# pureexe/deeparc-sfm

Hardware: AMD Instinct MI355X
Metric: M observations/sec residual+Jacobian; wall-clock/LM-iter at 1/2/4/8 GPUs (higher is better)
Workload: dtype f64; 1 GPU; c3_1kcam per GPU: 1000 cameras, 100000 points, 1000000 observations, BAL-shaped, eval pass = residual+Jacobian reduced into the JtJ/Jtr blocks; global_obs=1000000, parallelism=point-sharded x1, RCCL all-reduce of camera blocks

## Files before the change

### deeparc-sfm_amd/__init__.py

```python
from ._abi import (DAB_CONVERGENCE, DAB_E_INVALID, DAB_E_UNSUPPORTED, DAB_FAILURE, DAB_LINEAR_SOLVER_AUTO,
                   DAB_LINEAR_SOLVER_EXPLICIT_SCHUR, DAB_LINEAR_SOLVER_IMPLICIT_SCHUR_PCG, DAB_LOSS_CAUCHY,
                   DAB_LOSS_HUBER, DAB_LOSS_SOFT_L1, DAB_LOSS_TRIVIAL, DAB_NO_CONVERGENCE, LIB_PATH,
                   SIGNATURES, load_library, last_error)
from ._abi import DabCovarianceInfo, DabCovarianceIntrInfo, DabCovarianceOptions
from ._abi import DAB_INTR_CENTER, DAB_INTR_DISTORTION, DAB_INTR_FOCAL
from ._abi import DAB_EXT_ROTATION, DAB_EXT_TRANSLATION
from ._abi import DAB_SCHUR_DIRECT, DAB_SCHUR_PAIRS, DAB_SCHUR_TILES
from .core import (CONFIGS, Problem, Solver, covariance_options, options, point_sqrt_info_from_sigmas, solve,
                   sqrt_info_from_sigmas, synth, synth_config)

__all__ = [
    "CONFIGS", "Problem", "Solver", "options", "solve", "synth", "synth_config",
    "covariance_options", "DabCovarianceOptions", "DabCovarianceInfo", "DabCovarianceIntrInfo",
    "load_library", "last_error", "LIB_PATH", "SIGNATURES",
    "DAB_CONVERGENCE", "DAB_NO_CONVERGENCE", "DAB_FAILURE",
    "DAB_LINEAR_SOLVER_EXPLICIT_SCHUR", "DAB_LINEAR_SOLVER_IMPLICIT_SCHUR_PCG", "DAB_LINEAR_SOLVER_AUTO",
    "DAB_LOSS_TRIVIAL", "DAB_LOSS_HUBER", "DAB_LOSS_SOFT_L1", "DAB_LOSS_CAUCHY",
    "DAB_E_INVALID", "DAB_E_UNSUPPORTED",
    "DAB_INTR_CENTER", "DAB_INTR_FOCAL", "DAB_INTR_DISTORTION",
    "DAB_EXT_ROTATION", "DAB_EXT_TRANSLATION",
    "DAB_SCHUR_PAIRS", "DAB_SCHUR_TILES", "DAB_SCHUR_DIRECT",
    "sqrt_info_from_sigmas", "point_sqrt_info_from_sigmas",
]
```

### deeparc-sfm_amd/_abi.py

```python
import ctypes as C
import os

HERE = os.path.dirname(os.path.abspath(__file__))
LIB_PATH = os.path.join(HERE, "libdab.so")

DAB_OK = 0
DAB_LINEAR_SOLVER_EXPLICIT_SCHUR = 0
DAB_LINEAR_SOLVER_IMPLICIT_SCHUR_PCG = 1
DAB_LINEAR_SOLVER_AUTO = 2
DAB_CONVERGENCE = 0
DAB_NO_CONVERGENCE = 1
DAB_FAILURE = 2
TERMINATION = {0: "CONVERGENCE", 1: "NO_CONVERGENCE", 2: "FAILURE"}
DAB_E_INVALID = -1
DAB_E_UNSUPPORTED = -6
DAB_LOSS_TRIVIAL = 0
DAB_LOSS_HUBER = 1
DAB_LOSS_SOFT_L1 = 2
DAB_LOSS_CAUCHY = 3
DAB_INTR_CENTER = 1
DAB_INTR_FOCAL = 2
DAB_INTR_DISTORTION = 4
DAB_EXT_ROTATION = 0x07
DAB_EXT_TRANSLATION = 0x38
# ... 143 lines not shown
    "dab_eval_intr_priors": (C.c_int, [C.c_void_p, _dp, _dp]),
    "dab_get_intrinsics": (C.c_int, [C.c_void_p, _dp]),
    "dab_update_intrinsics": (C.c_int, [C.c_void_p, _dp]),
    "dab_eval_intrinsic_jacobians": (C.c_int, [C.c_void_p, _dp]),
    "dab_get_intrinsic_blocks": (C.c_int, [C.c_void_p, _ip, _dp]),
    "dab_covariance_options_init": (None, [C.POINTER(DabCovarianceOptions)]),
    "dab_covariance": (C.c_int, [C.c_void_p, C.POINTER(DabCovarianceOptions), _dp, _dp, _dp,
                                 C.POINTER(DabCovarianceInfo)]),
    "dab_covariance_intrinsics": (C.c_int, [C.c_void_p, C.POINTER(DabCovarianceOptions), _dp, _dp, _dp, _dp,
                                            C.POINTER(DabCovarianceInfo), C.POINTER(DabCovarianceIntrInfo)]),
    "dab_eval_residuals": (C.c_int, [C.c_void_p, _dp, _dp]),
    "dab_eval_jacobians": (C.c_int, [C.c_void_p, _dp, _dp]),
    "dab_filter": (C.c_int, [C.c_void_p, C.c_double, _dp, C.c_double, _u8p, _u8p, _ip, _ip]),
    "dab_dense_spd_solve": (C.c_int, [C.c_void_p, C.c_int, _dp, _dp, _dp, _dp]),
    "dab_bench_eval_pass": (C.c_int, [C.c_void_p, C.c_int, C.c_int]),
    "dab_sync": (C.c_int, [C.c_void_p]),
    "dab_bench_get_blocks": (C.c_int, [C.c_void_p, _ip, _ip, _dp, _dp, _dp, _dp, _dp]),
    "dab_bench_kernel_ms": (C.c_int, [C.c_void_p, _dp, _dp]),
    "dab_jacobian_bytes": (C.c_int, [C.c_void_p, _dp]),
    "dab_bench_pair_ms": (C.c_int, [C.c_void_p, _dp, _dp]),
    "dab_eval_schedule": (C.c_int, [C.c_void_p, _ip]),
    "dab_pcg_schedule": (C.c_int, [C.c_void_p, _ip]),
    "dab_comm_schedule": (C.c_int, [C.c_void_p, _ip]),
    "dab_synth_sizes": (C.c_int, [C.POINTER(DabSynthConfig), _ip, _ip, _ip, _ip]),
    "dab_synth_fill": (C.c_int, [C.POINTER(DabSynthConfig), C.POINTER(DabProblem), _u8p]),
}

_LIB = None


def load_library(path=None):
    global _LIB
    if _LIB is not None and path is None:
        return _LIB
    p = path or LIB_PATH
    if not os.path.exists(p):
        raise RuntimeError(
            f"libdab.so not found at {p}: build it with `make -C deeparc-sfm_amd` "
            "(hipcc --offload-arch=gfx950). There is no CPU fallback.")
    lib = C.CDLL(p)
    for name, (res, args) in SIGNATURES.items():
        fn = getattr(lib, name)
        fn.restype = res
        fn.argtypes = args
    if lib.dab_abi_version() != 2:
        raise RuntimeError("libdab ABI version mismatch")
# ... 16 lines not shown
```

### deeparc-sfm_amd/core.py

```python
import ctypes as C

import numpy as np

from . import _abi
from ._abi import (DabOptions, DabProblem, DabSummary, DabIteration, DabSynthConfig,
                   DabCovarianceOptions, DabCovarianceInfo, DabCovarianceIntrInfo, check, load_library)


def _ptr(a, ct):
    return a.ctypes.data_as(C.POINTER(ct)) if a is not None else None


class Problem:

    def __init__(self, obs_xy, obs_point, obs_ext0, obs_ext1, obs_intr, points, ext, intr,
                 intr_nf, intr_nk, ext_const=None, freeze_camera=False):
        self.obs_xy = np.ascontiguousarray(obs_xy, dtype=np.float64).reshape(-1, 2)
        self.obs_point = np.ascontiguousarray(obs_point, dtype=np.int32)
        self.obs_ext0 = np.ascontiguousarray(obs_ext0, dtype=np.int32)
        self.obs_ext1 = np.ascontiguousarray(obs_ext1, dtype=np.int32)
        self.obs_intr = np.ascontiguousarray(obs_intr, dtype=np.int32)
        self.points = np.ascontiguousarray(points, dtype=np.float64).reshape(-1, 3)
        self.ext = np.ascontiguousarray(ext, dtype=np.float64).reshape(-1, 6)
        self.intr = np.ascontiguousarray(intr, dtype=np.float64).reshape(-1, 6)
# ... 545 lines not shown
        return b.value

    def bench_pair_ms(self):
        a, b = C.c_double(), C.c_double()
        check(self.lib.dab_bench_pair_ms(self.h, C.byref(a), C.byref(b)), self.lib)
        return a.value, b.value

    def comm_p2p(self):
        f = C.c_int32()
        check(self.lib.dab_comm_schedule(self.h, C.byref(f)), self.lib)
        return int(f.value)

    def pcg_matrix_free(self):
        f = C.c_int32()
        check(self.lib.dab_pcg_schedule(self.h, C.byref(f)), self.lib)
        return int(f.value)

    def eval_fused(self):
        f = C.c_int32()
        check(self.lib.dab_eval_schedule(self.h, C.byref(f)), self.lib)
        return f.value


def sqrt_info_from_sigmas(sigma_w, sigma_t, n=None):
    def inv(sg):
        return 0.0 if sg is None or np.isinf(sg) else 1.0 / float(sg)
    a = np.diag([inv(sigma_w)] * 3 + [inv(sigma_t)] * 3)
    return a if n is None else np.repeat(a[None], int(n), axis=0)


def point_sqrt_info_from_sigmas(sigma, n=None):
    sg = [sigma] * 3 if sigma is None or np.ndim(sigma) == 0 else list(sigma)
    if len(sg) != 3:
        raise ValueError("sigma: a scalar or 3 values")
    a = np.diag([0.0 if v is None or np.isinf(v) else 1.0 / float(v) for v in sg])
    return a if n is None else np.repeat(a[None], int(n), axis=0)


def solve(problem, max_iteration=1000, max_second=3600, freeze_camera=False, device=0,
          verbose=False, loss=None, free_intrinsics=0, freeze_points=False, ext_priors=None, point_priors=None,
          intr_priors=None, ext_scalars_constant=None, **opt_kw):
    problem.freeze_camera = bool(freeze_camera)
    o = options(max_num_iterations=max_iteration, max_solver_time_in_seconds=float(max_second),
                minimizer_progress_to_stdout=int(verbose), **opt_kw)
    s = Solver(device)
    try:
# ... 19 lines not shown
```

### deeparc-sfm_amd/csrc/dab_handle.h

```cpp
#pragma once
#include <hip/hip_runtime.h>
#include <rccl/rccl.h>

#include <algorithm>
#include <limits>
#include <array>
#include <chrono>
#include <climits>
#include <cmath>
#include <cstdio>
#include <cstdlib>
#include <cstring>
#include <string>
#include <thread>
#include <vector>

#include "dab_devmem.h"
#include "dab_internal.h"
#include "dab_kernels.h"
#include "dab_p2p.h"
#include "dab_setup.h"

#define HIP_OK(expr)                                                                           \
  do {                                                                                         \
// ... 127 lines not shown
  S_SYNC,
  S_SYNC1,
  S_ZPRIOR,
  S_NSLOTS
};


template <class T, class A>
int upload(T** dptr, Dev& dev, const std::vector<T, A>& h, hipStream_t s) {
  CHECK_RC(dev.alloc(dptr, h.size()));
  if (!h.empty()) HIP_OK(hipMemcpyAsync(*dptr, h.data(), h.size() * sizeof(T), hipMemcpyHostToDevice, s));
  return 0;
}

struct Knobs {
  int chunk = 0;
  int xchunk = 0;
  int pair_eval = -1;
  int eval_wps = INT_MIN;
  int eval_fused = 1;
  int eval_split = 0;
  int pcg_fused = 1;
  int pcg_mf = 1;
  int cg_onewg = 0;
  int bench_sample = 8;
  int schur_tiles = 1;
  int tile_balance = 1;
  int tile_single = 1;
  int tile_minb = 2;
  int p2p = -1;
  int intr_border_lds = 1;
  int setup_host = 0;
  int eval_side = 0;
  int fused_tab = -1;
  int points_direct = 1;
  void read() {
    auto get = [](const char* name, int& out) {
      if (const char* e = getenv(name)) out = atoi(e);
    };
    get("DAB_CHUNK", chunk);
    get("DAB_XCHUNK", xchunk);
    get("DAB_PAIR_EVAL", pair_eval);
    get("DAB_EVAL_WPS", eval_wps);
    get("DAB_EVAL_FUSED", eval_fused);
    get("DAB_EVAL_SPLIT", eval_split);
    get("DAB_PCG_FUSED", pcg_fused);
    get("DAB_PCG_MF", pcg_mf);
    get("DAB_CG_ONEWG", cg_onewg);
    get("DAB_BENCH_SAMPLE", bench_sample);
    get("DAB_SCHUR_TILES", schur_tiles);
    get("DAB_TILE_BALANCE", tile_balance);
    get("DAB_TILE_MINB", tile_minb);
    get("DAB_TILE_SINGLE", tile_single);
    get("DAB_P2P", p2p);
    get("DAB_FUSED_TAB", fused_tab);
    get("DAB_SETUP_HOST", setup_host);
    get("DAB_INTR_BORDER_LDS", intr_border_lds);
    get("DAB_EVAL_SIDE", eval_side);
    get("DAB_POINTS_DIRECT", points_direct);
  }
  bool eval_side_ok() const {
#ifdef DAB_ABLATIONS
    return eval_side >= 0 && eval_side <= 7;
#else
    return eval_side == 0 || eval_side == 7;
#endif
  }
};

struct PhaseTimer {
// ... 35 lines not shown
  bool any_compose = false;
  std::vector<int> perm;
  std::vector<int> pt_of;
  std::vector<int> ext_col;
  int nchunk = 0, nxchunk = 0, ncross = 0, nblk = 0, nslice = 0;
  int max_seg_chunks = 1, max_xseg_chunks = 1;
  int NS = 0;
  long long npairs = 0;
  int lds = 0;
  bool schur_built = false;
  bool pcg_built = false;
  int nxlist = 0;
  std::vector<int> h_pt_ent_ptr;
  big_vec<int> h_ent_cam, h_ent_pos, h_ent_os;

  Dev dev{"problem buffers"};
  Dev setup_tmp{"set-up scratch"};
  Dev keep_dev{"kept buffers"};
  DevView view{};
  double loss_scale = 0.0;
  int4* d_obs_idx = nullptr;
  double2* d_obs_xy = nullptr;
  int* d_obs_e = nullptr;
  int4* d_cm_idx = nullptr;
  double2* d_cm_xy = nullptr;
  int4* d_x_idx = nullptr;
  double2* d_x_xy = nullptr;
  int *d_slice_off = nullptr, *d_pt_ent_ptr = nullptr, *d_ent_os = nullptr, *d_ent_cam = nullptr,
      *d_ent_pt = nullptr, *d_ent_pos = nullptr, *d_cm_pt = nullptr, *d_ext_col = nullptr;
  int *d_chunk_beg = nullptr, *d_seg_chunk = nullptr;
  int2* d_chunk_uni = nullptr;
  int uni_affine = 0, uni_ox = 0, uni_oi = 0;
  unsigned* d_arrivals = nullptr;
  int* d_chunk_lists = nullptr;
  ChunkLists chunks;
  int *d_xchunk_beg = nullptr, *d_xseg_chunk = nullptr;
  int2* d_cross_cam = nullptr;
  int2 *d_pairs = nullptr, *d_blk_cam = nullptr;
  int2* d_blk_zero = nullptr;
  int nzero = 0;
  int* d_blk_pair_beg = nullptr;
  double* d_intr = nullptr;
  std::vector<uint8_t> intr_mask;
  std::vector<uint8_t> intr_ref;
  bool intr_ref_union = false;
  std::vector<double> intr_host;
// ... 340 lines not shown
```

### deeparc-sfm_amd/csrc/dab_handle.hip

```cpp
#include <map>
#include <mutex>

#include "dab_handle.h"
#include "dab_warm.h"

using namespace dab;

namespace dab {
namespace {
std::mutex& cache_mu() {
  static std::mutex* m = new std::mutex();
  return *m;
}
std::map<int, std::vector<hipStream_t>>& stream_cache() {
  static auto* c = new std::map<int, std::vector<hipStream_t>>();
  return *c;
}
std::map<size_t, std::vector<void*>>& pinned_cache() {
  static auto* c = new std::map<size_t, std::vector<void*>>();
  return *c;
}
}
hipStream_t stream_take(int device) {
  {
// ... 329 lines not shown
  if (!h || !h->have_problem) return set_error(DAB_E_STATE, "no problem set");
  HIP_OK(hipSetDevice(h->device));
  if (points) {
    std::vector<double> pts((size_t)3 * h->NP);
    HIP_OK(hipMemcpyAsync(pts.data(), h->d_points, pts.size() * sizeof(double), hipMemcpyDeviceToHost, h->stream));
    HIP_OK(hipStreamSynchronize(h->stream));
    for (int i = 0; i < h->NP; ++i)
      for (int k = 0; k < 3; ++k) points[3 * (size_t)h->pt_of[i] + k] = pts[3 * (size_t)i + k];
  }
  if (ext) {
    HIP_OK(hipMemcpyAsync(ext, h->d_ext, sizeof(double) * 6 * (size_t)h->E, hipMemcpyDeviceToHost, h->stream));
    HIP_OK(hipStreamSynchronize(h->stream));
  }
  return 0;
}

extern "C" int dab_comm_schedule(dab_handle* h, int32_t* p2p) {
  clear_error();
  if (!h || !p2p) return set_error(DAB_E_INVALID, "null argument");
  *p2p = (h->p2p_main || h->p2p_comm) ? 1 : 0;
  return 0;
}

extern "C" int dab_pcg_schedule(dab_handle* h, int32_t* matrix_free) {
  clear_error();
  if (!h || !h->have_problem || !matrix_free) return set_error(DAB_E_STATE, "no problem set");
  *matrix_free = h->pcg_built && h->mf ? (h->mf32 ? 2 : 1) : 0;
  return 0;
}

extern "C" int dab_eval_schedule(dab_handle* h, int32_t* fused) {
  clear_error();
  if (!h || !h->have_problem || !fused) return set_error(DAB_E_STATE, "no problem set");
  *fused = h->fused ? (h->fused_split ? 2 : 1) : 0;
  return 0;
}
```

### deeparc-sfm_amd/csrc/dab_k_step.hip

```cpp
#include <hip/hip_runtime.h>

#include <algorithm>

#include "dab_kernels.h"
#include "dab_reduce.h"
#include "dab_rows.h"
#include "dab_warm.h"
#include "dab_wave.h"

namespace dab {

__global__ __launch_bounds__(256) void k_point_factor(DevView v, const double* __restrict__ V,
                                                      const double* __restrict__ g,
                                                      const double* __restrict__ sp, StepScalars sc,
                                                      double* __restrict__ L, double* __restrict__ q,
                                                      int* __restrict__ fail) {
  const int p = blockIdx.x * blockDim.x + threadIdx.x;
  if (p >= v.NP) return;
  const size_t NPs = (size_t)v.NP;
  const double s0 = sp[p], s1 = sp[NPs + p], s2 = sp[2 * NPs + p];
  double v00 = s0 * V[p] * s0, v01 = s0 * V[NPs + p] * s1, v02 = s0 * V[2 * NPs + p] * s2;
  double v11 = s1 * V[3 * NPs + p] * s1, v12 = s1 * V[4 * NPs + p] * s2, v22 = s2 * V[5 * NPs + p] * s2;
  auto lmd = [&](double d) {
    d = fmin(fmax(d, sc.min_diag), sc.max_diag);
    const double D = sqrt(d / sc.radius);
    return D * D;
  };
  v00 += lmd(v00);
  v11 += lmd(v11);
  v22 += lmd(v22);
  bool ok = v00 > 0.0;
// ... 367 lines not shown
#pragma unroll
      for (int slot = 0; slot < 2; ++slot) {
        const int e = slot ? id.z : id.y;
        const int c = e >= 0 ? v.ext_col[e] : -1;
        if (c < 0) continue;
        double y[18];
        load_yplane(Ypm + slot * 18 * NS, NS, (size_t)s, y);
#pragma unroll
        for (int a = 0; a < 6; ++a) {
          const double ycv = yc[6 * c + a];
          r[0] -= y[3 * a] * ycv;
          r[1] -= y[3 * a + 1] * ycv;
          r[2] -= y[3 * a + 2] * ycv;
        }
      }
    }
  }
  const double* pu = PU + 6 * (size_t)p;
  dp[p] = -(pu[0] * r[0] + pu[1] * r[1] + pu[2] * r[2]);
  dp[NPs + p] = -(pu[3] * r[1] + pu[4] * r[2]);
  dp[2 * NPs + p] = -(pu[5] * r[2]);
}

void launch_backsub(hipStream_t s, const DevView& v, const double* PU, const double* q, YBufs Y,
                    const double* yc, double* delta_p) {
  if (v.NP <= 0) return;
  const int g = grid_for(v.NP, 256, 1 << 20);
  if (Y.f32) k_backsub<float><<<g, 256, 0, s>>>(v, PU, q, (const float*)Y.pm, yc, delta_p);
  else k_backsub<double><<<g, 256, 0, s>>>(v, PU, q, (const double*)Y.pm, yc, delta_p);
}

__global__ __launch_bounds__(256) void k_axpy_points(int NP, const double* __restrict__ x,
                                                     const double* __restrict__ d,
                                                     double* __restrict__ xc, double* __restrict__ partial) {
  double acc[2] = {0.0, 0.0};
  const size_t NPs = (size_t)NP;
  for (int i = blockIdx.x * blockDim.x + threadIdx.x; i < 3 * NP; i += gridDim.x * blockDim.x) {
    const int p = i / 3, k = i - 3 * (i / 3);
    const double xv = x[i];
    const double c = xv + d[k * NPs + p];
    xc[i] = c;
    const double dd = xv - c;
    acc[0] += dd * dd;
    acc[1] += c * c;
  }
  block_reduce_store<2>(acc, partial + 2 * (size_t)blockIdx.x);
}

void launch_axpy_points(hipStream_t s, int NP, const double* x, const double* d, double* xc,
                        double* partial, int grid) {
// ... 61 lines not shown
```

### deeparc-sfm_amd/csrc/dab_kernels.h

```cpp
#pragma once
#include <string>
#include <hip/hip_runtime.h>

#include <cstdint>

#include "../../include/dab.h"

namespace dab {

#define DAB_LOSS_SWITCH(loss_, ...)                                                          \
  switch (loss_) {                                                                           \
    case DAB_LOSS_HUBER: { constexpr int LOSS = DAB_LOSS_HUBER; __VA_ARGS__; } break;         \
    case DAB_LOSS_SOFT_L1: { constexpr int LOSS = DAB_LOSS_SOFT_L1; __VA_ARGS__; } break;     \
    case DAB_LOSS_CAUCHY: { constexpr int LOSS = DAB_LOSS_CAUCHY; __VA_ARGS__; } break;       \
    default: { constexpr int LOSS = DAB_LOSS_TRIVIAL; __VA_ARGS__; } break;                   \
  }

constexpr int kCamTab = 32;
constexpr int kIntr = 8;
constexpr int kYRec = 18;

struct YBufs {
  void* cm;
  void* pm;
// ... 26 lines not shown
  int E;
  int NC;
  int NE;
  int NI;
  int nslice;
  int any_comp;
  int uni_affine;
  int uni_ox, uni_oi;
  const int4* obs_idx;
  const double2* obs_xy;
  const int4* cm_idx;
  const double2* cm_xy;
  const int* slice_off;
  const int* pt_ent_ptr;
  const int* ent_os;
  const int* ent_cam;
  const int* ent_pt;
  const int* ent_pos;
  const int* cm_pt;
  const int* ext_col;
  const double* intr;
  const int2* chunk_uni;
  const int* obs_e;
  int loss;
  double loss_a, loss_b, loss_c;
};

struct ChunkLists {
  int nchunk = 0, nuni = 0, ngen = 0;
  const int* uni = nullptr;
  const int* gen = nullptr;
};

void launch_cam_tables(hipStream_t s, int E, const double* ext, double* camtab);
void launch_eval_points(hipStream_t s, const DevView& v, const double* points, const double* ext,
                        const double* camtab, double* V, double* g, double* partial, unsigned* arrivals,
                        double* cost, unsigned long long* costfx, unsigned long long* fx_next, int grid, int wps);
inline bool eval_points_fx(int wps) { return wps <= -100 && (-wps - 100) / 1000 != 64; }
bool eval_points_needs_camtab(int wps);
bool eval_points_lds_fits(int E);
constexpr int kLdsCams = 1024;
void launch_jacobian_full(hipStream_t s, const DevView& v, const double* points,
                          const double* camtab, double* r, double* Jfull);
void launch_residual(hipStream_t s, const DevView& v, const double* points, const double* camtab,
                     double* r_out , double* partial , int grid);
void launch_filter(hipStream_t s, const DevView& v, const double* points, const double* camtab, double eb,
// ... 161 lines not shown
                          double* cost);
void launch_zprior_candidate(hipStream_t s, int n, const int2* idx, const double* rec, const double* intr,
                             const double* intr_c, const double* dz, double* model);
void launch_zprior_eval(hipStream_t s, int n, const int2* idx, const double* rec, const double* intr, double* res);

enum { kPcgRunning = 0, kPcgSuccess = 1, kPcgNoConvergence = 2, kPcgFailure = 3 };
struct PcgState {
  double rho, Q0, alpha, eta, norm_b, pad[3];
  int iter, status, min_iter, max_iter;
};
void launch_pcg_diag_rhs_partial(hipStream_t s, const DevView& v, int nchunk, const int* chunk_beg,
                                 const int* run, YBufs Y, const double* q, double* partial);
void launch_pcg_setup(hipStream_t s, int NC, const double* ug, const double* scale_c, StepScalars sc,
                      const double* red, double* Ad, double* Minv, double* bvec, double* x, double* r,
                      int* fail);
void launch_pcg_init(hipStream_t s, int NC, const double* bvec, const int* fail, PcgState* st, double eta,
                     int min_iter, int max_iter, const double* Minv, const double* r, double* z, double* p);
bool pcg_fused_fits(int NC);
int pcg_fused_grid(int NP, int ncu);
void launch_pcg_fused(hipStream_t s, const DevView& v, YBufs Y, const double* vec, double* partial, double* w,
                      int grid, const PcgState* st);
void launch_pcg_matvec_passes(hipStream_t s, const DevView& v, int nchunk, const int* chunk_beg, YBufs Y,
                              const double* vec, double* t, double* partial, const PcgState* st);
void launch_cg_update(hipStream_t s, int NC, int mode, const double* Ad, const double* w, const int* xptr,
                      const int* xlist, const int2* xcam, const double* X, const double* scale_c,
                      const double* bvec, double* p, double* q, double* x, double* r, PcgState* st,
                      const double* Minv, double* z, double* partial, unsigned* cnt,
                      const double* wpart = nullptr, int wpart_g = 0);
int cg_partial_size(int NC);
void launch_pcg_update(hipStream_t s, int NC, int mode, const double* Ad, const double* w, const int* xptr,
                       const int* xlist, const int2* xcam, const double* X, const double* scale_c,
                       const double* bvec, double* p, double* q, double* x, double* r, PcgState* st,
                       const double* Minv, double* z);

bool mf_schur_fits(int NC, int E, int NI);
int mf_grid(int NP, int ncu);
void launch_mf_product(hipStream_t s, const DevView& v, const double* points, const double* camtab,
                       const double* scale_c, const double* PU, const double* vec, double* partial, double* w,
                       int grid, const PcgState* st);
void launch_mf_product32(hipStream_t s, const DevView& v, const double* points, const double* camtab,
                         const double* scale_c, const double* PU, const double* vec, double* partial, double* w,
                         int grid, const PcgState* st);
void launch_mf_backsub(hipStream_t s, const DevView& v, const double* points, const double* camtab,
                       const double* scale_c, const double* PU, const double* q, const double* yc, double* dp,
                       int grid);
void launch_mf_diag_rhs(hipStream_t s, const DevView& v, int nchunk, const int* run_beg, const int4* run_rec,
// ... 43 lines not shown
```

### deeparc-sfm_amd/csrc/dab_pcg.hip

```cpp
#include <hip/hip_runtime.h>

#include <algorithm>
#include <cstdlib>

#include <cfloat>

#include "dab_kernels.h"
#include "dab_warm.h"
#include "dab_wave.h"

namespace dab {

namespace {

constexpr int kOneWG = 1024;

__device__ __forceinline__ double wg_sum(double v, double* sh) {
  v = wave_sum_lane63(v);
  const int lane = threadIdx.x & 63, w = threadIdx.x >> 6;
  __syncthreads();
  if (lane == 63) sh[w] = v;
  __syncthreads();
  double t = 0.0;
  for (int i = 0; i < (int)(blockDim.x >> 6); ++i) t += sh[i];
  return t;
}

__device__ __forceinline__ bool zero_or_inf(double x) { return x == 0.0 || isinf(x); }

__device__ __forceinline__ int up6(int a, int b) { return a * 6 - (a * (a - 1)) / 2 + (b - a); }

}
// ... 223 lines not shown
      if (c < 0) continue;
      double y[18];
      load_yplane(Ypm + slot * 18 * NS, NS, (size_t)s, y);
      const double2* v2 = reinterpret_cast<const double2*>(vec + 6 * (size_t)c);
      double vc[6];
#pragma unroll
      for (int q = 0; q < 3; ++q) {
        const double2 w = v2[q];
        vc[2 * q] = w.x;
        vc[2 * q + 1] = w.y;
      }
#pragma unroll
      for (int a = 0; a < 6; ++a) {
        t0 += y[3 * a] * vc[a];
        t1 += y[3 * a + 1] * vc[a];
        t2 += y[3 * a + 2] * vc[a];
      }
    }
  }
  reinterpret_cast<double2*>(t)[2 * (size_t)p] = make_double2(t0, t1);
  reinterpret_cast<double2*>(t)[2 * (size_t)p + 1] = make_double2(t2, 0.0);
}

constexpr int kFuseCams = 160;
constexpr int kFuseBlock = 256;
template <class YT>
__global__ __launch_bounds__(kFuseBlock) void k_pcg_fused(DevView v, const YT* __restrict__ Ypm,
                                                          const double* __restrict__ vec,
                                                          double* __restrict__ partial, const PcgState* st) {
  extern __shared__ double accs[];
  if (st->status != kPcgRunning) return;
  const int NC6 = 6 * v.NC, w = threadIdx.x >> 6;
  for (int i = threadIdx.x; i < (kFuseBlock / 64) * NC6; i += blockDim.x) accs[i] = 0.0;
  __syncthreads();
  double* acc = accs + w * NC6;
  const size_t NS = (size_t)v.N;
  for (int p = blockIdx.x * blockDim.x + threadIdx.x; p < v.NP; p += gridDim.x * blockDim.x) {
    const int sl = p >> 6, lane = p & 63;
    const int off = v.slice_off[sl], len = (v.slice_off[sl + 1] - off) >> 6;
    double t0 = 0.0, t1 = 0.0, t2 = 0.0;
    for (int k = 0; k < len; ++k) {
      const int s = off + 64 * k + lane;
      const int4 id = v.obs_idx[s];
      if (id.x < 0) continue;
#pragma unroll
      for (int slot = 0; slot < 2; ++slot) {
// ... 408 lines not shown

void launch_pcg_init(hipStream_t s, int NC, const double* bvec, const int* fail, PcgState* st, double eta,
                     int min_iter, int max_iter, const double* Minv, const double* r, double* z, double* p) {
  k_pcg_init<<<1, kOneWG, 0, s>>>(NC, bvec, fail, st, eta, min_iter, max_iter, Minv, r, z, p);
}


bool pcg_fused_fits(int NC) { return NC > 0 && NC <= kFuseCams; }
int pcg_fused_grid(int NP, int ncu) { return std::max(1, std::min((NP + kFuseBlock - 1) / kFuseBlock, 4 * ncu)); }

void launch_pcg_fused(hipStream_t s, const DevView& v, YBufs Y, const double* vec, double* partial, double* w,
                      int grid, const PcgState* st) {
  const int NC6 = 6 * v.NC;
  const size_t lds = sizeof(double) * (kFuseBlock / 64) * NC6;
  if (Y.f32) k_pcg_fused<float><<<grid, kFuseBlock, lds, s>>>(v, (const float*)Y.pm, vec, partial, st);
  else k_pcg_fused<double><<<grid, kFuseBlock, lds, s>>>(v, (const double*)Y.pm, vec, partial, st);
  k_pcg_fused_final<<<NC6, 256, 0, s>>>(grid, NC6, partial, w, st);
}

void launch_pcg_fused_final(hipStream_t s, int grid, int NC6, const double* partial, double* w, const PcgState* st) {
  k_pcg_fused_final<<<NC6, 256, 0, s>>>(grid, NC6, partial, w, st);
}

void launch_pcg_matvec_passes(hipStream_t s, const DevView& v, int nchunk, const int* chunk_beg, YBufs Y,
                              const double* vec, double* t, double* partial, const PcgState* st) {
  const int g = grid_for(v.NP, 256, 1 << 20);
  if (Y.f32) {
    if (v.NP > 0) k_pcg_point_pass<float><<<g, 256, 0, s>>>(v, (const float*)Y.pm, vec, t, st);
    if (nchunk > 0)
      k_pcg_cam_pass<float><<<nchunk, kRedBlock, 0, s>>>(v, chunk_beg, (const float*)Y.cm, t, partial, st);
  } else {
    if (v.NP > 0) k_pcg_point_pass<double><<<g, 256, 0, s>>>(v, (const double*)Y.pm, vec, t, st);
    if (nchunk > 0)
      k_pcg_cam_pass<double><<<nchunk, kRedBlock, 0, s>>>(v, chunk_beg, (const double*)Y.cm, t, partial, st);
  }
}

void launch_cg_update(hipStream_t s, int NC, int mode, const double* Ad, const double* w, const int* xptr,
                      const int* xlist, const int2* xcam, const double* X, const double* scale_c,
                      const double* bvec, double* p, double* q, double* x, double* r, PcgState* st,
                      const double* Minv, double* z, double* partial, unsigned* cnt, const double* wpart,
                      int wpart_g) {
  if (NC <= 0) return;
  const int L = xptr ? 64 : 1;
  const int gq = (NC + kCgBlock / L - 1) / (kCgBlock / L), gx = (NC + kCgBlock - 1) / kCgBlock;
  if (mode != 2)
    k_cg_q<<<gq, kCgBlock, 0, s>>>(NC, mode, L, Ad, w, xptr, xlist, xcam, X, scale_c, bvec, p, q, x, r, st, partial, cnt,
                                   L == 64 ? wpart : nullptr, wpart_g);
  else
    k_cg_q<<<gq, kCgBlock, 0, s>>>(NC, 2, L, Ad, w, xptr, xlist, xcam, X, scale_c, bvec, p, q, x, r, st, partial, cnt,
                                   L == 64 ? wpart : nullptr, wpart_g);
  const int fold_p = 6 * NC <= 2048;
  k_cg_xr<<<gx, kCgBlock, 0, s>>>(NC, mode, bvec, p, q, x, r, Minv, z, st, partial, cnt, fold_p);
  if (mode != 1 && !fold_p) k_cg_p<<<(6 * NC + 255) / 256, 256, 0, s>>>(6 * NC, z, p, st);
}
// ... 13 lines not shown
```

### deeparc-sfm_amd/csrc/dab_problem.hip

```cpp
#include "dab_handle.h"

using namespace dab;

static size_t pair_piece(size_t n, int most) {
  const size_t m = (size_t)std::max(1, most), parts = std::max<size_t>(1, (n + m - 1) / m);
  return std::max<size_t>(1, (n + parts - 1) / parts);
}

static int validate(const dab_problem* p) {
  if (!p) return set_error(DAB_E_INVALID, "null problem");
  if (p->num_obs < 0 || p->num_points < 0 || p->num_ext < 0 || p->num_intr < 0)
    return set_error(DAB_E_INVALID, "negative size");
  if (p->num_obs > 0 && (!p->obs_xy || !p->obs_point || !p->obs_ext0 || !p->obs_ext1 || !p->obs_intr))
    return set_error(DAB_E_INVALID, "null observation array");
  if ((p->num_points > 0 && !p->points) || (p->num_ext > 0 && !p->ext) ||
      (p->num_intr > 0 && (!p->intr || !p->intr_nf || !p->intr_nk)))
    return set_error(DAB_E_INVALID, "null parameter array");
  for (int i = 0; i < p->num_intr; ++i) {
    if (p->intr_nf[i] < 1 || p->intr_nf[i] > 2) return set_error(DAB_E_INVALID, "intr_nf must be 1 or 2");
    if (p->intr_nk[i] < 0 || p->intr_nk[i] > 2) return set_error(DAB_E_INVALID, "intr_nk must be 0, 1 or 2");
  }
  return 0;
}
static int validate_obs(const dab_problem* p) {
// ... 545 lines not shown
  v.uni_oi = h->uni_oi;
  v.obs_idx = h->d_obs_idx;
  v.obs_xy = h->d_obs_xy;
  v.cm_idx = h->d_cm_idx;
  v.cm_xy = h->d_cm_xy;
  v.chunk_uni = h->d_chunk_uni;
  v.slice_off = h->d_slice_off;
  v.pt_ent_ptr = h->d_pt_ent_ptr;
  v.ent_os = h->d_ent_os;
  v.ent_cam = h->d_ent_cam;
  v.ent_pt = h->d_ent_pt;
  v.ent_pos = h->d_ent_pos;
  v.cm_pt = h->d_cm_pt;
  v.ext_col = h->d_ext_col;
  v.intr = h->d_intr;
  h->fused = h->fused && fused_eval_fits(v, h->nchunk, h->chunks.ngen, h->ncross, h->ncu);
  v.obs_e = nullptr;
  h->d_obs_e = nullptr;
  if (h->fused) {
    CHECK_RC(d.alloc(&h->d_obs_e, (size_t)std::max(1, NS)));
    su_obs_e(s, NS, h->d_obs_idx, h->d_obs_e);
    HIP_OK(hipStreamSynchronize(s));
    v.obs_e = h->d_obs_e;
  }
  HIP_OK(hipStreamSynchronize(s));
  phase("upload");
  h->have_problem = true;
  return 0;
}
static bool setup_device_fits(dab_handle* h, const dab_problem* p) {
  if (h->world > 1) return false;
  const long long ncam = p->num_ext;
  return ncam * ncam + 1 < (1LL << 30) && (long long)p->num_obs * 2 < (1LL << 30);
}
static int setup_device(dab_handle* h, const dab_problem* p, PhaseTimer& phase) {
  hipStream_t s = h->stream;
  Dev& d = h->dev;
  Dev& tmp = h->setup_tmp;
  tmp.release();
  const int N = p->num_obs, NPT = p->num_points, E = p->num_ext;
  void* rtmp = nullptr;
  size_t rtmp_cap = 0;
  auto rp = [&](auto call) -> int {
    size_t bytes = 0;
    if (call(nullptr, &bytes) != 0) return set_error(DAB_E_DEVICE, "rocPRIM size query failed");
    if (bytes > rtmp_cap) {
// ... 1126 lines not shown
```

### deeparc-sfm_amd/csrc/dab_setup.h

```cpp
#pragma once
#include <hip/hip_runtime.h>

#include <cstddef>

namespace dab {

int su_sort_pairs(void* tmp, size_t* tmp_bytes, const int* kin, int* kout, const int* vin, int* vout, int n,
                  int end_bit, hipStream_t s);
int su_exclusive_scan(void* tmp, size_t* tmp_bytes, const int* in, int* out, int n, hipStream_t s);
int su_max(void* tmp, size_t* tmp_bytes, const int* in, int* out, int n, hipStream_t s);
int su_select_flagged_i(void* tmp, size_t* tmp_bytes, const int* in, const unsigned char* flags, int* out,
                        int* count, int n, hipStream_t s);
int su_rle(void* tmp, size_t* tmp_bytes, const int* in, int* unique, int* counts, int* nruns, int n, hipStream_t s);

void su_count(hipStream_t s, int N, const int* obs_point, const int* obs_ext0, const int* obs_ext1,
              const int* obs_intr, int num_points, int num_ext, int num_intr, int* pcount, int* eref, int* flags);
void su_point_keys(hipStream_t s, int num_points, const int* pcount, const int* maxcount, int* keys, int* vals,
                   int* nref);
void su_point_local(hipStream_t s, int NP, const int* pt_of, const int* pcount, int* pt_local, int* lcount);
void su_obs_keys(hipStream_t s, int N, const int* obs_point, const int* pt_local, int* keys, int* vals);
void su_slice_len(hipStream_t s, int nslice, int NP, const int* lcount, int* slen);
void su_slots(hipStream_t s, int NP, int nslice, const int* slice_off, const int* cnt, const int* lcount,
              const int* by_pt, const int* obs_ext0, const int* obs_ext1, const int* obs_intr, const double* obs_xy,
              const int* ext_col, int4* obs_idx, double2* obs_xy_out, int* perm, int* ne);
void su_entries(hipStream_t s, int NP, const int* slice_off, const int* lcount, const int4* obs_idx,
                const int* ext_col, const int* pt_ent_ptr, int* ent_os, int* ent_cam, int* ent_pt);
void su_bounds(hipStream_t s, int n, const int* sorted_keys, int nkeys, int* start);
void su_camera_major(hipStream_t s, int NE, const int* cam_ent, const int* ent_pt, const int* ent_os,
                     const int4* obs_idx, const double2* obs_xy, int* ent_pos, int* cm_pt, int4* cm_idx,
                     double2* cm_xy);
void su_runs(hipStream_t s, int NE, const int* pos_cam, const int* cm_pt, int* run);
void su_chunk_runs(hipStream_t s, int nchunk, const int* chunk_beg, const int* run, int* run_cnt);
void su_chunk_run_rec(hipStream_t s, int nchunk, const int* chunk_beg, const int* run, const int* cm_pt,
                      const int* pos_cam, const int* run_beg, int4* run_rec);
void su_chunk_uni(hipStream_t s, int nchunk, const int* chunk_beg, const int4* cm_idx, int slot_bit, int2* chunk_uni);
void su_cross_keys(hipStream_t s, int NS, const int4* obs_idx, const int* ext_col, int NC, int* keys, int* vals,
                   int* nvalid);
void su_cross_copy(hipStream_t s, int n, const int* slots, const int4* obs_idx, const double2* obs_xy,
                   int4* x_idx, double2* x_xy, unsigned char* touched);
void su_count_flags(hipStream_t s, int n, const unsigned char* flags, int* count);
void su_pair_intr(hipStream_t s, int n, const int4* x_idx, int* count);
void su_unpaired_flags(hipStream_t s, int NE, const int4* cm_idx, const int* ext_col, unsigned char* flags,
                       int* flags_i);
void su_gather_cm(hipStream_t s, int n, const int* sel, const int4* cm_idx, const double2* cm_xy, int4* out_idx,
                  double2* out_xy);
void su_obs_e(hipStream_t s, int NS, const int4* obs_idx, int* obs_e);
void su_points(hipStream_t s, int NP, const int* pt_of, const double* raw_points, double* points);
void su_iota(hipStream_t s, int n, int* out);
void su_gather_at(hipStream_t s, int n, const int* idx, const int* in, int* out);
void su_pair_count(hipStream_t s, int NP, const int* pt_ent_ptr, const int* ent_cam, int* cnt,
                   unsigned long long* total);
void su_pair_gen(hipStream_t s, int NP, const int* pt_ent_ptr, const int* ent_cam, const int* poff, int NC, int* keys,
                 int* vals, int2* ef);
void su_pair_gather(hipStream_t s, int n, const int* idx, const int2* ef, const int* ent_pos, int2* pairs);
void su_tile_sort(hipStream_t s, int NP, const int* pt_ent_ptr, const int* ent_cam, const int* ent_os, int2* sch,
                  int* m);
void su_tile_batch(hipStream_t s, int nbatch, int NC, const int* batch_pt, const int* batch_rec, const int* pt_ent_ptr,
                   const int2* sch, const int4* obs_idx, int hdr_bytes, unsigned char* hdr, int4* rec, int4* robs);
void su_tile_hits(hipStream_t s, int NP, int nb, const int* pt_ent_ptr, const int2* sch, int* hits);

}
```

### deeparc-sfm_amd/csrc/dab_setup.hip

```cpp
#include <hip/hip_runtime.h>

#include <cstring>
#include <rocprim/device/device_radix_sort.hpp>
#include <rocprim/device/device_reduce.hpp>
#include <rocprim/device/device_run_length_encode.hpp>
#include <rocprim/device/device_scan.hpp>
#include <rocprim/device/device_select.hpp>

#include "dab_kernels.h"
#include "dab_setup.h"
#include "dab_warm.h"

namespace dab {

namespace {
constexpr int kSuBlock = 256;
inline unsigned su_grid(long long n) { return (unsigned)std::max(1LL, std::min((n + kSuBlock - 1) / kSuBlock, 1LL << 20)); }

__device__ __forceinline__ int block_sum(int x, int* lds) {
  const int lane = threadIdx.x & 63, w = threadIdx.x >> 6;
#pragma unroll
  for (int o = 32; o > 0; o >>= 1) x += __shfl_xor(x, o);
  if (lane == 0) lds[w] = x;
  __syncthreads();
// ... 403 lines not shown
__global__ void k_su_gather_cm(int n, const int* __restrict__ sel, const int4* __restrict__ cm_idx,
                               const double2* __restrict__ cm_xy, int4* __restrict__ out_idx,
                               double2* __restrict__ out_xy) {
  for (long long i = blockIdx.x * (long long)blockDim.x + threadIdx.x; i < n; i += (long long)gridDim.x * blockDim.x) {
    const int j = sel[i];
    out_idx[i] = cm_idx[j];
    out_xy[i] = cm_xy[j];
  }
}
void su_gather_cm(hipStream_t s, int n, const int* sel, const int4* cm_idx, const double2* cm_xy, int4* out_idx,
                  double2* out_xy) {
  if (n > 0) k_su_gather_cm<<<su_grid(n), kSuBlock, 0, s>>>(n, sel, cm_idx, cm_xy, out_idx, out_xy);
}

__global__ void k_su_obs_e(int NS, const int4* __restrict__ obs_idx, int* __restrict__ obs_e) {
  for (long long i = blockIdx.x * (long long)blockDim.x + threadIdx.x; i < NS; i += (long long)gridDim.x * blockDim.x) {
    const int4 id = obs_idx[i];
    obs_e[i] = id.x >= 0 ? (id.y | (id.w << 16)) : -1;
  }
}
void su_obs_e(hipStream_t s, int NS, const int4* obs_idx, int* obs_e) {
  if (NS > 0) k_su_obs_e<<<su_grid(NS), kSuBlock, 0, s>>>(NS, obs_idx, obs_e);
}
__global__ void k_su_points(int NP, const int* __restrict__ pt_of, const double* __restrict__ raw,
                            double* __restrict__ points) {
  const int i = blockIdx.x * blockDim.x + threadIdx.x;
  if (i >= 3 * NP) return;
  const int l = i / 3, k = i - 3 * l;
  points[i] = raw[3 * (size_t)pt_of[l] + k];
}
void su_points(hipStream_t s, int NP, const int* pt_of, const double* raw_points, double* points) {
  if (NP > 0) k_su_points<<<su_grid(3LL * NP), kSuBlock, 0, s>>>(NP, pt_of, raw_points, points);
}
__global__ void k_su_iota(int n, int* __restrict__ out) {
  for (long long i = blockIdx.x * (long long)blockDim.x + threadIdx.x; i < n; i += (long long)gridDim.x * blockDim.x)
    out[i] = (int)i;
}
void su_iota(hipStream_t s, int n, int* out) {
  if (n > 0) k_su_iota<<<su_grid(n), kSuBlock, 0, s>>>(n, out);
}

__global__ void k_su_gather_at(int n, const int* __restrict__ idx, const int* __restrict__ in, int* __restrict__ out) {
  const int c = blockIdx.x * blockDim.x + threadIdx.x;
  if (c < n) out[c] = in[idx[c]];
}
void su_gather_at(hipStream_t s, int n, const int* idx, const int* in, int* out) {
// ... 163 lines not shown
```

### include/dab.h

```cpp
#ifndef DAB_H_
#define DAB_H_

#include <stdint.h>

#ifdef __cplusplus
extern "C" {
#endif

#define DAB_ABI_VERSION 2

#define DAB_OK 0
#define DAB_E_INVALID (-1)
#define DAB_E_DEVICE (-2)
#define DAB_E_NOMEM (-3)
#define DAB_E_STATE (-4)
#define DAB_E_COMM (-5)
#define DAB_E_UNSUPPORTED (-6)

typedef struct dab_problem {
  int32_t num_obs;
  int32_t num_points;
  int32_t num_ext;
  int32_t num_intr;
  const double* obs_xy;
// ... 184 lines not shown
  int32_t num_free_scalars;
  double border_ms;
  double reserved;
} dab_covariance_intr_info;

int dab_covariance_intrinsics(dab_handle* h, const dab_covariance_options* opt ,
                              double* point_cov, double* ext_cov, double* intr_cov, double* cam_full,
                              dab_covariance_info* info, dab_covariance_intr_info* zinfo);

int dab_dense_spd_solve(dab_handle* h, int n, const double* A, const double* b, double* x,
                        double* factor_ms);

int dab_bench_eval_pass(dab_handle* h, int with_assembly, int count);
int dab_sync(dab_handle* h);
int dab_bench_get_blocks(dab_handle* h, int32_t* num_free_ext, int32_t* num_cross, double* V, double* g,
                         double* ug, double* ux, double* cost);
int dab_bench_kernel_ms(dab_handle* h, double* jac_ms, double* assembly_ms);
int dab_jacobian_bytes(dab_handle* h, double* bytes);
int dab_bench_pair_ms(dab_handle* h, double* ms, double* bytes);
int dab_eval_schedule(dab_handle* h, int32_t* fused);
int dab_pcg_schedule(dab_handle* h, int32_t* matrix_free);
int dab_comm_schedule(dab_handle* h, int32_t* p2p);

typedef struct dab_synth_config {
  int32_t kind;
  int32_t num_cameras;
  int32_t num_arcs;
  int32_t num_rings;
  int32_t num_points;
  int32_t obs_per_point;
  uint64_t seed;
  uint64_t point_seed;
  double pixel_noise;
  double point_noise;
  double rot_noise;
  double trans_noise;
} dab_synth_config;

int dab_synth_sizes(const dab_synth_config* cfg, int32_t* num_obs, int32_t* num_points,
                    int32_t* num_ext, int32_t* num_intr);
int dab_synth_fill(const dab_synth_config* cfg, dab_problem* p, uint8_t* ext_const);

#ifdef __cplusplus
}
#endif
#endif
// ... 1 lines not shown
```

Before: 50220 M obs/s.

## Add software-pipelined point-row kernels for PCG matvec and back-substitution

Adds a register-level software pipeline that prefetches camera column indices and Y-block rows a few slices ahead in the PCG point pass and back-substitution kernels. A new precomputed slot_col array removes the per-observation obs_idx to ext_col indirection. This targets load latency in the PCG and back-substitution phase. The measured metric is the residual+Jacobian evaluation pass, which these kernels do not touch, so the main effect there is extra setup memory and more register pressure in the new kernels.

Result: no change. 50250 M obs/s, median of 2 (+0.1%).

```diff
diff --git a/deeparc-sfm_amd/__init__.py b/deeparc-sfm_amd/__init__.py
--- a/deeparc-sfm_amd/__init__.py
+++ b/deeparc-sfm_amd/__init__.py
@@ -6,8 +6,8 @@
 from ._abi import DAB_INTR_CENTER, DAB_INTR_DISTORTION, DAB_INTR_FOCAL
 from ._abi import DAB_EXT_ROTATION, DAB_EXT_TRANSLATION
 from ._abi import DAB_SCHUR_DIRECT, DAB_SCHUR_PAIRS, DAB_SCHUR_TILES
-from .core import (CONFIGS, Problem, Solver, covariance_options, options, point_sqrt_info_from_sigmas, solve,
-                   sqrt_info_from_sigmas, synth, synth_config)
+from .core import (CONFIGS, Problem, Solver, covariance_options, options, pcg_pipe_depths,
+                   point_sqrt_info_from_sigmas, solve, sqrt_info_from_sigmas, synth, synth_config)
 
 __all__ = [
     "CONFIGS", "Problem", "Solver", "options", "solve", "synth", "synth_config",
@@ -20,5 +20,5 @@
     "DAB_INTR_CENTER", "DAB_INTR_FOCAL", "DAB_INTR_DISTORTION",
     "DAB_EXT_ROTATION", "DAB_EXT_TRANSLATION",
     "DAB_SCHUR_PAIRS", "DAB_SCHUR_TILES", "DAB_SCHUR_DIRECT",
-    "sqrt_info_from_sigmas", "point_sqrt_info_from_sigmas",
+    "sqrt_info_from_sigmas", "point_sqrt_info_from_sigmas", "pcg_pipe_depths",
 ]
diff --git a/deeparc-sfm_amd/_abi.py b/deeparc-sfm_amd/_abi.py
--- a/deeparc-sfm_amd/_abi.py
+++ b/deeparc-sfm_amd/_abi.py
@@ -189,6 +189,7 @@
     "dab_eval_schedule": (C.c_int, [C.c_void_p, _ip]),
     "dab_pcg_schedule": (C.c_int, [C.c_void_p, _ip]),
     "dab_comm_schedule": (C.c_int, [C.c_void_p, _ip]),
+    "dab_pcg_pipe_depths": (C.c_int, [_ip, _ip]),
     "dab_synth_sizes": (C.c_int, [C.POINTER(DabSynthConfig), _ip, _ip, _ip, _ip]),
     "dab_synth_fill": (C.c_int, [C.POINTER(DabSynthConfig), C.POINTER(DabProblem), _u8p]),
 }
diff --git a/deeparc-sfm_amd/core.py b/deeparc-sfm_amd/core.py
--- a/deeparc-sfm_amd/core.py
+++ b/deeparc-sfm_amd/core.py
@@ -591,6 +591,12 @@
         return f.value
 
 
+def pcg_pipe_depths():
+    a, b = C.c_int32(), C.c_int32()
+    check(load_library().dab_pcg_pipe_depths(C.byref(a), C.byref(b)), load_library())
+    return int(a.value), int(b.value)
+
+
 def sqrt_info_from_sigmas(sigma_w, sigma_t, n=None):
     def inv(sg):
         return 0.0 if sg is None or np.isinf(sg) else 1.0 / float(sg)
diff --git a/deeparc-sfm_amd/csrc/dab_handle.h b/deeparc-sfm_amd/csrc/dab_handle.h
--- a/deeparc-sfm_amd/csrc/dab_handle.h
+++ b/deeparc-sfm_amd/csrc/dab_handle.h
@@ -173,6 +173,7 @@
   int eval_split = 0;
   int pcg_fused = 1;
   int pcg_mf = 1;
+  int pcg_pipe = 1;
   int cg_onewg = 0;
   int bench_sample = 8;
   int schur_tiles = 1;
@@ -197,6 +198,7 @@
     get("DAB_EVAL_SPLIT", eval_split);
     get("DAB_PCG_FUSED", pcg_fused);
     get("DAB_PCG_MF", pcg_mf);
+    get("DAB_PCG_PIPE", pcg_pipe);
     get("DAB_CG_ONEWG", cg_onewg);
     get("DAB_BENCH_SAMPLE", bench_sample);
     get("DAB_SCHUR_TILES", schur_tiles);
@@ -278,6 +280,7 @@
   int4* d_obs_idx = nullptr;
   double2* d_obs_xy = nullptr;
   int* d_obs_e = nullptr;
+  int* d_slot_col = nullptr;
   int4* d_cm_idx = nullptr;
   double2* d_cm_xy = nullptr;
   int4* d_x_idx = nullptr;
diff --git a/deeparc-sfm_amd/csrc/dab_handle.hip b/deeparc-sfm_amd/csrc/dab_handle.hip
--- a/deeparc-sfm_amd/csrc/dab_handle.hip
+++ b/deeparc-sfm_amd/csrc/dab_handle.hip
@@ -375,6 +375,12 @@
   return 0;
 }
 
+extern "C" int dab_pcg_pipe_depths(int32_t* rows, int32_t* rows2) {
+  if (rows) *rows = pcg_pipe_depth(0);
+  if (rows2) *rows2 = pcg_pipe_depth(1);
+  return 0;
+}
+
 extern "C" int dab_pcg_schedule(dab_handle* h, int32_t* matrix_free) {
   clear_error();
   if (!h || !h->have_problem || !matrix_free) return set_error(DAB_E_STATE, "no problem set");
diff --git a/deeparc-sfm_amd/csrc/dab_k_step.hip b/deeparc-sfm_amd/csrc/dab_k_step.hip
--- a/deeparc-sfm_amd/csrc/dab_k_step.hip
+++ b/deeparc-sfm_amd/csrc/dab_k_step.hip
@@ -7,6 +7,7 @@
 #include "dab_rows.h"
 #include "dab_warm.h"
 #include "dab_wave.h"
+#include "dab_ypipe.h"
 
 namespace dab {
 
@@ -420,10 +421,38 @@
   dp[2 * NPs + p] = -(pu[5] * r[2]);
 }
 
+template <class YT, int NSLOT>
+__global__ __launch_bounds__(256) void k_backsub_pipe(DevView v, const double* __restrict__ PU,
+                                                      const double* __restrict__ q, const YT* __restrict__ Ypm,
+                                                      const double* __restrict__ yc, double* __restrict__ dp) {
+  const int p = blockIdx.x * blockDim.x + threadIdx.x;
+  if (p >= v.NP) return;
+  const size_t NPs = (size_t)v.NP;
+  const double2 qa = reinterpret_cast<const double2*>(q)[2 * (size_t)p];
+  double r[3] = {qa.x, qa.y, q[4 * (size_t)p + 2]};
+  if (yc)
+    point_rows_pipe<YT, NSLOT, NSLOT == 1 ? kPipeD : kPipeD2, true, false>(
+        v, Ypm, yc, __builtin_amdgcn_readfirstlane(p >> 6), p & 63, r);
+  const double* pu = PU + 6 * (size_t)p;
+  dp[p] = -(pu[0] * r[0] + pu[1] * r[1] + pu[2] * r[2]);
+  dp[NPs + p] = -(pu[3] * r[1] + pu[4] * r[2]);
+  dp[2 * NPs + p] = -(pu[5] * r[2]);
+}
+
 void launch_backsub(hipStream_t s, const DevView& v, const double* PU, const double* q, YBufs Y,
                     const double* yc, double* delta_p) {
   if (v.NP <= 0) return;
   const int g = grid_for(v.NP, 256, 1 << 20);
+  if (v.slot_col) {
+    if (v.any_comp) {
+      if (Y.f32) k_backsub_pipe<float, 2><<<g, 256, 0, s>>>(v, PU, q, (const float*)Y.pm, yc, delta_p);
+      else k_backsub_pipe<double, 2><<<g, 256, 0, s>>>(v, PU, q, (const double*)Y.pm, yc, delta_p);
+    } else {
+      if (Y.f32) k_backsub_pipe<float, 1><<<g, 256, 0, s>>>(v, PU, q, (const float*)Y.pm, yc, delta_p);
+      else k_backsub_pipe<double, 1><<<g, 256, 0, s>>>(v, PU, q, (const double*)Y.pm, yc, delta_p);
+    }
+    return;
+  }
   if (Y.f32) k_backsub<float><<<g, 256, 0, s>>>(v, PU, q, (const float*)Y.pm, yc, delta_p);
   else k_backsub<double><<<g, 256, 0, s>>>(v, PU, q, (const double*)Y.pm, yc, delta_p);
 }
diff --git a/deeparc-sfm_amd/csrc/dab_kernels.h b/deeparc-sfm_amd/csrc/dab_kernels.h
--- a/deeparc-sfm_amd/csrc/dab_kernels.h
+++ b/deeparc-sfm_amd/csrc/dab_kernels.h
@@ -72,6 +72,7 @@
   const double* intr;
   const int2* chunk_uni;
   const int* obs_e;
+  const int* slot_col;
   int loss;
   double loss_a, loss_b, loss_c;
 };
@@ -279,6 +280,7 @@
                       int grid, const PcgState* st);
 void launch_pcg_matvec_passes(hipStream_t s, const DevView& v, int nchunk, const int* chunk_beg, YBufs Y,
                               const double* vec, double* t, double* partial, const PcgState* st);
+int pcg_pipe_depth(int which);
 void launch_cg_update(hipStream_t s, int NC, int mode, const double* Ad, const double* w, const int* xptr,
                       const int* xlist, const int2* xcam, const double* X, const double* scale_c,
                       const double* bvec, double* p, double* q, double* x, double* r, PcgState* st,
diff --git a/deeparc-sfm_amd/csrc/dab_pcg.hip b/deeparc-sfm_amd/csrc/dab_pcg.hip
--- a/deeparc-sfm_amd/csrc/dab_pcg.hip
+++ b/deeparc-sfm_amd/csrc/dab_pcg.hip
@@ -8,6 +8,7 @@
 #include "dab_kernels.h"
 #include "dab_warm.h"
 #include "dab_wave.h"
+#include "dab_ypipe.h"
 
 namespace dab {
 
@@ -277,6 +278,20 @@
   reinterpret_cast<double2*>(t)[2 * (size_t)p + 1] = make_double2(t2, 0.0);
 }
 
+template <class YT, int NSLOT>
+__global__ __launch_bounds__(256) void k_pcg_point_pass_pipe(DevView v, const YT* __restrict__ Ypm,
+                                                             const double* __restrict__ vec,
+                                                             double* __restrict__ t, const PcgState* st) {
+  if (st->status != kPcgRunning) return;
+  const int p = blockIdx.x * blockDim.x + threadIdx.x;
+  if (p >= v.NP) return;
+  double acc[3] = {0.0, 0.0, 0.0};
+  point_rows_pipe<YT, NSLOT, NSLOT == 1 ? kPipeD : kPipeD2, false, true>(
+      v, Ypm, vec, __builtin_amdgcn_readfirstlane(p >> 6), p & 63, acc);
+  reinterpret_cast<double2*>(t)[2 * (size_t)p] = make_double2(acc[0], acc[1]);
+  reinterpret_cast<double2*>(t)[2 * (size_t)p + 1] = make_double2(acc[2], 0.0);
+}
+
 constexpr int kFuseCams = 160;
 constexpr int kFuseBlock = 256;
 template <class YT>
@@ -731,15 +746,30 @@
   k_pcg_fused_final<<<NC6, 256, 0, s>>>(grid, NC6, partial, w, st);
 }
 
+static void launch_point_pass_pipe(hipStream_t s, const DevView& v, int g, YBufs Y, const double* vec, double* t,
+                                   const PcgState* st) {
+  if (v.NP <= 0) return;
+  if (v.any_comp) {
+    if (Y.f32) k_pcg_point_pass_pipe<float, 2><<<g, 256, 0, s>>>(v, (const float*)Y.pm, vec, t, st);
+    else k_pcg_point_pass_pipe<double, 2><<<g, 256, 0, s>>>(v, (const double*)Y.pm, vec, t, st);
+  } else {
+    if (Y.f32) k_pcg_point_pass_pipe<float, 1><<<g, 256, 0, s>>>(v, (const float*)Y.pm, vec, t, st);
+    else k_pcg_point_pass_pipe<double, 1><<<g, 256, 0, s>>>(v, (const double*)Y.pm, vec, t, st);
+  }
+}
+
+int pcg_pipe_depth(int which) { return which == 0 ? kPipeD : kPipeD2; }
+
 void launch_pcg_matvec_passes(hipStream_t s, const DevView& v, int nchunk, const int* chunk_beg, YBufs Y,
                               const double* vec, double* t, double* partial, const PcgState* st) {
   const int g = grid_for(v.NP, 256, 1 << 20);
+  if (v.slot_col) launch_point_pass_pipe(s, v, g, Y, vec, t, st);
   if (Y.f32) {
-    if (v.NP > 0) k_pcg_point_pass<float><<<g, 256, 0, s>>>(v, (const float*)Y.pm, vec, t, st);
+    if (v.NP > 0 && !v.slot_col) k_pcg_point_pass<float><<<g, 256, 0, s>>>(v, (const float*)Y.pm, vec, t, st);
     if (nchunk > 0)
       k_pcg_cam_pass<float><<<nchunk, kRedBlock, 0, s>>>(v, chunk_beg, (const float*)Y.cm, t, partial, st);
   } else {
-    if (v.NP > 0) k_pcg_point_pass<double><<<g, 256, 0, s>>>(v, (const double*)Y.pm, vec, t, st);
+    if (v.NP > 0 && !v.slot_col) k_pcg_point_pass<double><<<g, 256, 0, s>>>(v, (const double*)Y.pm, vec, t, st);
     if (nchunk > 0)
       k_pcg_cam_pass<double><<<nchunk, kRedBlock, 0, s>>>(v, chunk_beg, (const double*)Y.cm, t, partial, st);
   }
diff --git a/deeparc-sfm_amd/csrc/dab_problem.hip b/deeparc-sfm_amd/csrc/dab_problem.hip
--- a/deeparc-sfm_amd/csrc/dab_problem.hip
+++ b/deeparc-sfm_amd/csrc/dab_problem.hip
@@ -591,6 +591,13 @@
     su_obs_e(s, NS, h->d_obs_idx, h->d_obs_e);
     HIP_OK(hipStreamSynchronize(s));
     v.obs_e = h->d_obs_e;
+  }
+  v.slot_col = nullptr;
+  h->d_slot_col = nullptr;
+  if (h->knobs.pcg_pipe != 0) {
+    CHECK_RC(d.alloc(&h->d_slot_col, (size_t)std::max(1, NS) * (v.any_comp ? 2 : 1)));
+    su_slot_col(s, NS, v.any_comp != 0, h->d_obs_idx, h->d_ext_col, h->d_slot_col);
+    v.slot_col = h->d_slot_col;
   }
   HIP_OK(hipStreamSynchronize(s));
   phase("upload");
diff --git a/deeparc-sfm_amd/csrc/dab_setup.h b/deeparc-sfm_amd/csrc/dab_setup.h
--- a/deeparc-sfm_amd/csrc/dab_setup.h
+++ b/deeparc-sfm_amd/csrc/dab_setup.h
@@ -46,6 +46,7 @@
                   double2* out_xy);
 void su_obs_e(hipStream_t s, int NS, const int4* obs_idx, int* obs_e);
 void su_points(hipStream_t s, int NP, const int* pt_of, const double* raw_points, double* points);
+void su_slot_col(hipStream_t s, int NS, bool two, const int4* obs_idx, const int* ext_col, int* slot_col);
 void su_iota(hipStream_t s, int n, int* out);
 void su_gather_at(hipStream_t s, int n, const int* idx, const int* in, int* out);
 void su_pair_count(hipStream_t s, int NP, const int* pt_ent_ptr, const int* ent_cam, int* cnt,
diff --git a/deeparc-sfm_amd/csrc/dab_setup.hip b/deeparc-sfm_amd/csrc/dab_setup.hip
--- a/deeparc-sfm_amd/csrc/dab_setup.hip
+++ b/deeparc-sfm_amd/csrc/dab_setup.hip
@@ -449,6 +449,25 @@
 void su_obs_e(hipStream_t s, int NS, const int4* obs_idx, int* obs_e) {
   if (NS > 0) k_su_obs_e<<<su_grid(NS), kSuBlock, 0, s>>>(NS, obs_idx, obs_e);
 }
+template <int W>
+__global__ void k_su_slot_col(int NS, const int4* __restrict__ obs_idx, const int* __restrict__ ext_col,
+                              int* __restrict__ slot_col) {
+  for (long long i = blockIdx.x * (long long)blockDim.x + threadIdx.x; i < NS; i += (long long)gridDim.x * blockDim.x) {
+    const int4 id = obs_idx[i];
+    const int c0 = id.x >= 0 && id.y >= 0 ? ext_col[id.y] : -1;
+    if (W == 2) {
+      const int c1 = id.x >= 0 && id.z >= 0 ? ext_col[id.z] : -1;
+      reinterpret_cast<int2*>(slot_col)[i] = make_int2(c0, c1);
+    } else {
+      slot_col[i] = c0;
+    }
+  }
+}
+void su_slot_col(hipStream_t s, int NS, bool two, const int4* obs_idx, const int* ext_col, int* slot_col) {
+  if (NS <= 0) return;
+  if (two) k_su_slot_col<2><<<su_grid(NS), kSuBlock, 0, s>>>(NS, obs_idx, ext_col, slot_col);
+  else k_su_slot_col<1><<<su_grid(NS), kSuBlock, 0, s>>>(NS, obs_idx, ext_col, slot_col);
+}
 __global__ void k_su_points(int NP, const int* __restrict__ pt_of, const double* __restrict__ raw,
                             double* __restrict__ points) {
   const int i = blockIdx.x * blockDim.x + threadIdx.x;
diff --git a/deeparc-sfm_amd/csrc/dab_ypipe.h b/deeparc-sfm_amd/csrc/dab_ypipe.h
--- /dev/null
+++ b/deeparc-sfm_amd/csrc/dab_ypipe.h
@@ -0,0 +1,90 @@
+#pragma once
+#include <hip/hip_runtime.h>
+
+#include "dab_kernels.h"
+
+namespace dab {
+
+#ifndef DAB_PIPE_D
+#define DAB_PIPE_D 3
+#endif
+constexpr int kPipeD = DAB_PIPE_D;
+constexpr int kPipeD2 = 1;
+
+template <class YT, int NSLOT, int D, bool SUB, bool V2>
+__device__ __forceinline__ void point_rows_pipe(const DevView& v, const YT* __restrict__ Ypm,
+                                                const double* __restrict__ vec, int sl, int lane,
+                                                double (&acc)[3]) {
+  constexpr int R = D + 1;
+  constexpr int RC = 2 * R;
+  const size_t NS = (size_t)v.N;
+  const int off = v.slice_off[sl], len = (v.slice_off[sl + 1] - off) >> 6;
+  if (len <= 0) return;
+  int col[RC][NSLOT];
+  YT y[R][NSLOT][18];
+  double g[R][NSLOT][6];
+  const auto load_col = [&](int k, int (&c)[NSLOT]) {
+    const size_t s = (size_t)(off + 64 * min(k, len - 1) + lane);
+    if (NSLOT == 2) {
+      const int2 cc = reinterpret_cast<const int2*>(v.slot_col)[s];
+      c[0] = cc.x;
+      c[NSLOT - 1] = cc.y;
+    } else {
+      c[0] = v.slot_col[s];
+    }
+  };
+  const auto load_row = [&](int k, const int (&c)[NSLOT], YT (&yy)[NSLOT][18], double (&gg)[NSLOT][6]) {
+    const size_t s = (size_t)(off + 64 * min(k, len - 1) + lane);
+#pragma unroll
+    for (int slot = 0; slot < NSLOT; ++slot) {
+      const double* vc = vec + 6 * (size_t)max(c[slot], 0);
+      if (V2) {
+#pragma unroll
+        for (int q = 0; q < 3; ++q) {
+          const double2 w = reinterpret_cast<const double2*>(vc)[q];
+          gg[slot][2 * q] = w.x;
+          gg[slot][2 * q + 1] = w.y;
+        }
+      } else {
+#pragma unroll
+        for (int a = 0; a < 6; ++a) gg[slot][a] = vc[a];
+      }
+      const YT* yp = Ypm + slot * 18 * NS + s;
+#pragma unroll
+      for (int j = 0; j < 18; ++j) yy[slot][j] = yp[j * NS];
+    }
+  };
+#pragma unroll
+  for (int u = 0; u < RC - 1; ++u) load_col(u, col[u]);
+#pragma unroll
+  for (int u = 0; u < D; ++u) load_row(u, col[u], y[u], g[u]);
+  for (int k0 = 0; k0 < len; k0 += RC) {
+#pragma unroll
+    for (int u = 0; u < RC; ++u) {
+      const int k = k0 + u;
+      if (k >= len) return;
+      load_col(k + RC - 1, col[(u + RC - 1) % RC]);
+      load_row(k + D, col[(u + D) % RC], y[(u + D) % R], g[(u + D) % R]);
+#pragma unroll
+      for (int slot = 0; slot < NSLOT; ++slot) {
+        if (col[u][slot] < 0) continue;
+        const YT(&yy)[18] = y[u % R][slot];
+        const double(&vc)[6] = g[u % R][slot];
+#pragma unroll
+        for (int a = 0; a < 6; ++a) {
+          if (SUB) {
+            acc[0] -= (double)yy[3 * a] * vc[a];
+            acc[1] -= (double)yy[3 * a + 1] * vc[a];
+            acc[2] -= (double)yy[3 * a + 2] * vc[a];
+          } else {
+            acc[0] += (double)yy[3 * a] * vc[a];
+            acc[1] += (double)yy[3 * a + 1] * vc[a];
+            acc[2] += (double)yy[3 * a + 2] * vc[a];
+          }
+        }
+      }
+    }
+  }
+}
+
+}
diff --git a/include/dab.h b/include/dab.h
--- a/include/dab.h
+++ b/include/dab.h
@@ -230,6 +230,7 @@
 int dab_pcg_schedule(dab_handle* h, int32_t* matrix_free);
 int dab_comm_schedule(dab_handle* h, int32_t* p2p);
 
+int dab_pcg_pipe_depths(int32_t* rows, int32_t* rows2);
 typedef struct dab_synth_config {
   int32_t kind;
   int32_t num_cameras;
```
